# kingdwd/nlp-filter

Hardware: AMD Instinct MI355X
Metric: Gauss-Newton collocation-point updates/sec (higher is better)
Workload: dtype f64; 1 GPU; C2 van_der_pol: n=2, m=1, full_state p=2, N=100 (P=101, d=202), T=10, M=101; global_batch=1024, batch_per_gpu=1024, parallelism=dp1 (independent trajectories; RCCL broadcast of constants only)

## Files before the change

### nlp-filter_amd/csrc/mhe_core.h

```cpp
#pragma once
#include <hip/hip_runtime.h>
#include <math.h>
#include <stdint.h>
#include <stdlib.h>

#include "mhe.h"
#include "mhe_models.h"
#include "mhe_wave.h"

namespace mhe {

typedef double d4 __attribute__((ext_vector_type(4)));

#ifndef MHE_GN_MINW
#define MHE_GN_MINW 4
#endif
#ifndef MHE_NW
#define MHE_NW 8
#endif
constexpr int NW = MHE_NW;
constexpr int NTHREADS = NW * 64;
constexpr int MAX_NT = 13;
constexpr int MAX_SLOTS = (MAX_NT * (MAX_NT - 1) / 2 + NW - 1) / NW;

enum Mode { MODE_SOLVE = 0, MODE_ASSEMBLE = 1, MODE_LINSOLVE = 2, MODE_COV = 3 };

extern int g_opt_big_right_looking;
extern int g_opt_smem_pad;
extern int g_opt_lsm_group;

struct ConstLayout {
  size_t D, Dt, Phi, PhiT, cw, Qw, Pw, Rw, Cc, DA, DB, DAc, DBc, total;
};

__host__ __device__ inline size_t align256(size_t x) { return (x + 255) & ~size_t(255); }

constexpr size_t CONST_HEADER = 256;

__host__ __device__ inline ConstLayout const_layout(int P, int M, int n, int p, int NT) {
  ConstLayout L;
  size_t o = CONST_HEADER;
  const size_t ntiles = size_t(NT) * (NT + 1) / 2;
  L.D = o;    o = align256(o + sizeof(double) * P * P);
  L.Dt = o;   o = align256(o + sizeof(double) * P * P);
  L.Phi = o;  o = align256(o + sizeof(double) * M * P);
  L.PhiT = o; o = align256(o + sizeof(double) * M * P);
  L.cw = o;   o = align256(o + sizeof(double) * P);
  L.Qw = o;   o = align256(o + sizeof(double) * n * n);
  L.Pw = o;   o = align256(o + sizeof(double) * n * n);
  L.Rw = o;   o = align256(o + sizeof(double) * M * p * p);
  L.Cc = o;   o = align256(o + sizeof(double) * ntiles * 256);
  L.DA = o;   o = align256(o + sizeof(double) * ntiles * 256);
  L.DB = o;   o = align256(o + sizeof(double) * ntiles * 256);
  L.DAc = o;  o = align256(o + sizeof(double) * ntiles * 64);
  L.DBc = o;  o = align256(o + sizeof(double) * ntiles * 64);
  L.total = o;
  return L;
}

struct SmemLayout {
  int Xs, Vs, FtV, Es, FtE, GE, G, LAM, BV, YV, PB, HB, BAND, ZT, DT, RED, ROWM, UN, XO, ACT, GV, ZP, total;
};

__host__ __device__ inline int rnd2(int x) { return (x + 1) & ~1; }

constexpr int DTS = 272;
constexpr int LIS = 17;
constexpr int UNITS = 68;
constexpr int MFMA_NEG_A = 1;
__host__ __device__ constexpr int unit_row(int i) { return (i & 1) ? 51 - i : 16 - i; }

__host__ __device__ inline SmemLayout smem_layout(int P, int M, int n, int NT, bool nonlinear, bool bounded = false,
                                                  bool sb = false, bool cov = false) {
  SmemLayout S;
  int o = 0;
  const int dp = 16 * NT;
  S.Xs = o;   o += rnd2(P * n);
  S.Vs = o;   o += rnd2(P * n);
  S.FtV = o;  o += rnd2(P * n);
  S.Es = o;   o += rnd2(P * n * n);
  S.FtE = o;  o += rnd2(P * n * n);
  S.GE = o;   o += rnd2(M * n);
  S.G = o;    o += nonlinear ? rnd2(M * n * n) : 0;
  S.LAM = o;  o += rnd2(P * n);
  S.BV = o;   o += dp;
  S.YV = o;   o += dp;
  S.PB = o;   o += (sb ? 2 : 1) * (NT - 1) * 256;
  S.HB = o;   o += sb ? 2 * 256 : 0;
  S.BAND = o; o += sb ? (NT - 1) * 256 : 0;
  S.ZT = o;   o += sb ? 256 : 0;
  S.DT = o;   o += NT * DTS;
  S.RED = o;  o += 4 * NW + 8;
  S.ROWM = o; o += NW * 8;
  S.UN = o;   o += UNITS;
  S.XO = o;   o += bounded ? rnd2(P * n) : 0;
  S.ACT = o;  o += bounded ? dp / 2 : 0;
  S.GV = o;   o += bounded ? dp : 0;
  S.ZP = o;   o += cov ? dp * 16 : 0;
  S.total = o;
  return S;
}

struct GnArgs {
  const char* cbuf;
  int P, M, d, NT, ntiles, q, has_prior;
  int idx[8];
  double alpha;
  const double* X0;
  double* Xout;
  const double* U;
  long long ustride;
  const double* Y;
  const double* PAR;
  long long pstride;
  const double* x0;
  double* cost;
  int* iters;
  int* status;
  int max_iter;
  double tol;
  double* Hout;
  double* gout;
  const double* Hin;
  const double* gin;
  double* dout;
  unsigned long long* dbg;
  double huber_delta;
  int n_bounds;
  unsigned long long tag;
  int bidx[8];
  double blb[8], bub[8];
  double dpar[8];
  const double* Rw;
  long long rwstride;
  const double* PhiQ;
  int nq;
  double* cov;
  const double* md;
  long long mdstride;
  const double* Pw;
  long long pwstride;
  const double* Z0;
  double* Zout;
  double* lam;
  int nz, nc;
};

__device__ __forceinline__ const double* prior_weight(const GnArgs& a, const ConstLayout& CL, int b) {
  return a.Pw ? a.Pw + (long long)b * a.pwstride : (const double*)(a.cbuf + CL.Pw);
}

#ifdef MHE_DIAG
#define DIAG_DECL unsigned long long _dg[16] = {}; unsigned long long _dt = __builtin_amdgcn_s_memtime();
#define DIAG_MARK(i) do { const unsigned long long _n = __builtin_amdgcn_s_memtime(); _dg[i] += _n - _dt; _dt = _n; } while (0)
#define DIAG_FLUSH(b) do { if (threadIdx.x == 0 && a.dbg) for (int _i = 0; _i < 16; ++_i) a.dbg[(b) * 16 + _i] = _dg[_i]; } while (0)
#define DIAG_FDECL unsigned long long* _dg, unsigned long long& _dt
#define DIAG_FARGS _dg, _dt
#else
#define DIAG_DECL
#define DIAG_MARK(i) do { } while (0)
#define DIAG_FLUSH(b) do { } while (0)
#define DIAG_FDECL int
#define DIAG_FARGS 0
#endif

#ifndef MHE_KO
#define MHE_KO 0
#endif
#define KO(bit) ((MHE_KO >> (bit)) & 1)

__device__ __forceinline__ double readlane_d(double v, int lane) {
  const long long b = __double_as_longlong(v);
  const int lo = __builtin_amdgcn_readlane((int)b, lane);
  const int hi = __builtin_amdgcn_readlane((int)(b >> 32), lane);
  return __longlong_as_double(((long long)hi << 32) | (unsigned int)lo);
}

typedef unsigned int mhe_u2 __attribute__((ext_vector_type(2)));
__device__ __forceinline__ __amdgpu_buffer_rsrc_t cbuf_rsrc(const char* cbuf, size_t bytes) {
  return __builtin_amdgcn_make_buffer_rsrc((void*)cbuf, (short)0, (int)bytes, 0x00020000);
}
__device__ __forceinline__ double bload(__amdgpu_buffer_rsrc_t r, int voff, int soff) {
  const mhe_u2 v = __builtin_amdgcn_raw_buffer_load_b64(r, voff, soff, 0);
  return __builtin_bit_cast(double, v);
}


__device__ __forceinline__ void spread_dblock(double v, double (&o)[4]) {
  const double ev = dpp_d<0xA0>(v);
  const double od = dpp_d<0xF5>(v);
  const long long be = __double_as_longlong(ev), bo = __double_as_longlong(od);
  const auto el = __builtin_amdgcn_permlane16_swap((int)be, (int)be, false, false);
  const auto eh = __builtin_amdgcn_permlane16_swap((int)(be >> 32), (int)(be >> 32), false, false);
  const auto ol = __builtin_amdgcn_permlane16_swap((int)bo, (int)bo, false, false);
  const auto oh = __builtin_amdgcn_permlane16_swap((int)(bo >> 32), (int)(bo >> 32), false, false);
  o[0] = __longlong_as_double(((long long)eh[0] << 32) | (unsigned int)el[0]);
  o[2] = __longlong_as_double(((long long)eh[1] << 32) | (unsigned int)el[1]);
  o[1] = __longlong_as_double(((long long)oh[0] << 32) | (unsigned int)ol[0]);
  o[3] = __longlong_as_double(((long long)oh[1] << 32) | (unsigned int)ol[1]);
}

__device__ __forceinline__ double wave_max(double v) {
  v = fmax(v, dpp_d<0xB1>(v));
  v = fmax(v, dpp_d<0x4E>(v));
  v = fmax(v, dpp_d<0x141>(v));
  v = fmax(v, dpp_d<0x140>(v));
  v = pair_combine<1, true>(v);
  return pair_combine<2, true>(v);
}

template <bool SW = false>
__device__ __forceinline__ void block_reduce2(double* red, double& a, double& b, bool is_max) {
  const int lane = threadIdx.x & 63;
  int wave = threadIdx.x >> 6;
  if constexpr (SW) wave = __builtin_amdgcn_readfirstlane(wave);
  a = is_max ? wave_max(a) : wave_sum(a);
  b = is_max ? wave_max(b) : wave_sum(b);
  if (lane == 0) {
    red[2 * wave] = a;
    red[2 * wave + 1] = b;
  }
  __syncthreads();
  double ra = red[0], rb = red[1];
#pragma unroll
  for (int w = 1; w < NW; ++w) {
    ra = is_max ? fmax(ra, red[2 * w]) : ra + red[2 * w];
    rb = is_max ? fmax(rb, red[2 * w + 1]) : rb + red[2 * w + 1];
  }
  __syncthreads();
  a = ra;
  b = rb;
}

__device__ __forceinline__ int make_slot_table(int wave, int lane, int NT) {
  const int u = wave + NW * lane;
  if (lane >= MAX_SLOTS || u >= NT * (NT - 1) / 2) return -1;
  int J = 0, base = 0;
  while (u >= base + (NT - 1 - J)) {
    base += NT - 1 - J;
    ++J;
  }
  return (J + 1 + (u - base)) | (J << 16);
}

__device__ __forceinline__ int tile_index(int I, int J, int NT) { return J * NT - J * (J - 1) / 2 + (I - J); }

__device__ __forceinline__ int slot_ij(int stab, int s) { return __builtin_amdgcn_readlane(stab, s); }

__device__ __forceinline__ int slot_start(int j, int wave, int NT) {
  const int base = j * (NT - 1) - j * (j - 1) / 2;
  return base > wave ? (base - wave + NW - 1) / NW : 0;
}

struct ChainMap {
  unsigned short ij[NW][MAX_SLOTS];
  unsigned char pre[NW][16];
  unsigned char rows[MAX_NT][NW];
};

constexpr ChainMap make_chain_map(int NT) {
  ChainMap m = {};
  int rem[NW] = {}, nslot[NW] = {}, colc[MAX_NT][NW] = {};
  for (int w = 0; w < NW; ++w) {
    rem[w] = MAX_SLOTS;
    for (int s = 0; s < MAX_SLOTS; ++s) m.ij[w][s] = 0xffff;
  }
  int need = NT * (NT - 1) / 2 - (NW - 1) * MAX_SLOTS;
  for (int J = 0; J + 1 < NT; ++J) {
// ... 44 lines not shown

constexpr bool CHAIN_NW = NW == 8;
struct ChainMaps {
  ChainMap nt[MAX_NT + 1];
};
constexpr ChainMaps make_chain_maps() {
  ChainMaps a = {};
  for (int NT = 1; CHAIN_NW && NT <= MAX_NT; ++NT) a.nt[NT] = make_chain_map(NT);
  return a;
}

constexpr bool chain_map_ok(const ChainMap& m, int NT) {
  int seen[MAX_NT][MAX_NT] = {};
  for (int w = 0; w < NW; ++w) {
    int last = -1, rowc[MAX_NT] = {};
    bool ended = false;
    for (int s = 0; s < MAX_SLOTS; ++s) {
      const int v = m.ij[w][s];
      if (v == 0xffff) {
        ended = true;
        continue;
      }
      const int I = v & 0xff, J = v >> 8;
      if (ended || I <= J || I >= NT) return false;
      if ((J << 8 | I) <= last) return false;
      last = J << 8 | I;
      ++seen[I][J];
      ++rowc[J];
    }
    for (int J = 0; J + 1 < NT; ++J) {
      if (rowc[J] > (NT - 1 - J + NW - 1) / NW || rowc[J] != m.rows[J][w]) return false;
      if (m.pre[w][J + 1] - m.pre[w][J] != rowc[J]) return false;
    }
    if (m.pre[w][0] != 0) return false;
  }
  for (int I = 0; I < NT; ++I)
    for (int J = 0; J < NT; ++J)
      if (seen[I][J] != (I > J ? 1 : 0)) return false;
  for (int k = 0; k + 1 < NT; ++k) {
    for (int w = 1; w < NW; ++w) {
      int t0 = 0, tw = 0;
      for (int J = k + 1; J + 1 < NT; ++J) t0 += m.rows[J][0], tw += m.rows[J][w];
      if (tw < t0) return false;
    }
  }
  return true;
}
constexpr bool chain_maps_ok(const ChainMaps& a) {
  for (int NT = 1; NT <= MAX_NT; ++NT)
    if (!chain_map_ok(a.nt[NT], NT)) return false;
  return true;
}
constexpr ChainMaps CHAIN_MAPS_H = make_chain_maps();
static_assert(!CHAIN_NW || chain_maps_ok(CHAIN_MAPS_H),
              "panel-aware slot map: tile ownership, slot limit, row spread or slot order");
static __constant__ ChainMaps CHAIN_MAPS = CHAIN_MAPS_H;

constexpr int CHL_PRE = 16;
__device__ __forceinline__ int make_slot_table_chain(int wave, int lane, int NT) {
  const ChainMap& m = CHAIN_MAPS.nt[NT];
  if (lane >= CHL_PRE + 16) return -1;
  if (lane >= CHL_PRE) return m.pre[wave][lane - CHL_PRE];
  if (lane >= MAX_SLOTS) return -1;
  const int v = m.ij[wave][lane];
  return v == 0xffff ? -1 : (v & 0xff) | ((v >> 8) << 16);
}

__device__ __forceinline__ void init_units(double* un) {
  if (threadIdx.x < 64)
    for (int e = threadIdx.x; e < UNITS; e += 64) un[e] = (e == 16 || e == 51) ? 1.0 : 0.0;
}

template <int SLOTS = MAX_SLOTS>
__device__ __forceinline__ void init_rowmask(int* rowm, int wave, int lane, int stab) {
  unsigned m = 0;
#pragma unroll
  for (int s = 0; s < SLOTS; ++s) {
    const int IJ = slot_ij(stab, s);
    if (IJ >= 0 && (IJ & 0xffff) == lane) m |= 1u << s;
  }
  if (lane < 16) rowm[wave * 16 + lane] = (int)m;
}

constexpr int TPR = NW >= 8 ? 4 : 2;

__device__ __forceinline__ int opaque_tid() {
  int t = threadIdx.x;
  asm volatile("" : "+v"(t));
  return t;
}

template <int n>
__device__ __forceinline__ void dot_rows_part(const double* __restrict__ Mt, int ld, int row, int len, int part,
                                              const double* __restrict__ Xs, double (&acc)[n]) {
#pragma unroll
  for (int c = 0; c < n; ++c) acc[c] = 0.0;
  int j = part;
#pragma unroll 1
  for (; j + TPR * 7 < len; j += TPR * 8) {
    double m[8];
#pragma unroll
    for (int u = 0; u < 8; ++u) m[u] = Mt[(j + TPR * u) * ld + row];
#pragma unroll
    for (int u = 0; u < 8; ++u)
#pragma unroll
      for (int c = 0; c < n; ++c) acc[c] += m[u] * Xs[(j + TPR * u) * n + c];
  }
  for (; j < len; j += TPR) {
    const double mv = Mt[j * ld + row];
#pragma unroll
    for (int c = 0; c < n; ++c) acc[c] += mv * Xs[j * n + c];
  }
  static_assert(TPR == 4, "quad reductions below assume 4 lanes per row");
#pragma unroll
  for (int c = 0; c < n; ++c) acc[c] += dpp_d<0xB1>(acc[c]);
#pragma unroll
  for (int c = 0; c < n; ++c) acc[c] += dpp_d<0x4E>(acc[c]);
}

template <class DYN, bool HUBER = false>
__device__ __forceinline__ double node_row(const GnArgs& a, const ConstLayout& CL, const SmemLayout& SL, double* sm,
                                           int b, int k, const double (&dx)[DYN::n]) {
  constexpr int n = DYN::n, m = DYN::m;
  const double* cw = (const double*)(a.cbuf + CL.cw);
  const double* Qw = (const double*)(a.cbuf + CL.Qw);
  const double* Xs = sm + SL.Xs;
  double cost = 0.0;
  {
    double xk[n], uk[m > 0 ? m : 1], f[n], F[n * n];
#pragma unroll
    for (int c = 0; c < n; ++c) xk[c] = Xs[k * n + c];
    if (m > 0) {
      const double* U = a.U + (long long)b * a.ustride + (long long)k * m;
#pragma unroll
      for (int c = 0; c < m; ++c) uk[c] = U[c];
    }
    DYN::eval(xk, uk, a.dpar, f, F);
    double W[n], V[n];
#pragma unroll
    for (int c = 0; c < n; ++c) W[c] = a.alpha * dx[c] - f[c];
    const double ck = cw[k];
    double E[n * n];
    if constexpr (HUBER) {
      const double dl = a.huber_delta;
#pragma unroll
      for (int r = 0; r < n; ++r) {
        const double q = Qw[r * n + r];
        const double sr = sqrt(1.0 + W[r] * W[r] / (dl * dl));
        const double lam = ck * (q / sr);
        V[r] = lam * W[r];
        cost += ck * (2.0 * q * dl * dl * (sr - 1.0));
        sm[SL.LAM + k * n + r] = lam;
#pragma unroll
        for (int c = 0; c < n; ++c) E[r * n + c] = lam * F[r * n + c];
      }
    } else {
#pragma unroll
      for (int r = 0; r < n; ++r) {
        double s = 0.0;
#pragma unroll
        for (int c = 0; c < n; ++c) s += Qw[r * n + c] * W[c];
        V[r] = ck * s;
        cost += W[r] * V[r];
      }
#pragma unroll
      for (int r = 0; r < n; ++r)
#pragma unroll
// ... 110 lines not shown
      }
    }
    double* GE = sm + SL.GE + i * n;
#pragma unroll
    for (int c = 0; c < n; ++c) {
      double s = 0.0;
#pragma unroll
      for (int r = 0; r < p; ++r) s += H[r * n + c] * Re[r];
      GE[c] = s;
    }
    if (!MEAS::LINEAR) {
      double* G = sm + SL.G + i * n * n;
      double RH[p * n];
#pragma unroll
      for (int r = 0; r < p; ++r)
#pragma unroll
        for (int c = 0; c < n; ++c) {
          double s = 0.0;
#pragma unroll
          for (int t = 0; t < p; ++t) s += R[r * p + t] * H[t * n + c];
          RH[r * n + c] = s;
        }
#pragma unroll
      for (int r = 0; r < n; ++r)
#pragma unroll
        for (int c = 0; c < n; ++c) {
          double s = 0.0;
#pragma unroll
          for (int t = 0; t < p; ++t) s += H[t * n + r] * RH[t * n + c];
          G[r * n + c] = s;
        }
    }
  }
  return cost;
}

template <class DYN, class MEAS, bool NOISE = false, bool MHUBER = false>
__device__ __forceinline__ double meas_phase(const GnArgs& a, const ConstLayout& CL, const SmemLayout& SL, double* sm, int b,
                                             double* nzp = nullptr) {
  constexpr int n = DYN::n;
  const double* PhiT = (const double*)(a.cbuf + CL.PhiT);
  const double* Xs = sm + SL.Xs;
  double cost = 0.0;
  const int tid = opaque_tid();
  const int part = tid % TPR;
  for (int i0 = 0; i0 < a.M; i0 += NTHREADS / TPR) {
    const int i = i0 + tid / TPR;
    const int ii = i < a.M ? i : a.M - 1;
    double xi[n];
    dot_rows_part<n>(PhiT, a.M, ii, a.P, part, Xs, xi);
    if (part || i >= a.M) continue;
    cost += meas_row<DYN, MEAS, NOISE, MHUBER>(a, CL, SL, sm, b, i, xi, nzp);
  }
  return cost;
}

__device__ __forceinline__ double row_pair_sum(double v) {
  const long long b = __double_as_longlong(v);
  const auto l = __builtin_amdgcn_permlane16_swap((int)b, (int)b, false, false);
  const auto h = __builtin_amdgcn_permlane16_swap((int)(b >> 32), (int)(b >> 32), false, false);
  return __longlong_as_double(((long long)h[0] << 32) | (unsigned int)l[0]) +
         __longlong_as_double(((long long)h[1] << 32) | (unsigned int)l[1]);
}
__device__ __forceinline__ double upper_half(double v) {
  const long long b = __double_as_longlong(v);
  const auto l = __builtin_amdgcn_permlane32_swap((int)b, (int)b, false, false);
  const auto h = __builtin_amdgcn_permlane32_swap((int)(b >> 32), (int)(b >> 32), false, false);
  return __longlong_as_double(((long long)h[1] << 32) | (unsigned int)l[1]);
}

template <class DYN, class MEAS, bool HUBER = false, bool NOISE = false, bool MHUBER = false, bool SKIP = false>
__device__ __forceinline__ double node_meas_phase(const GnArgs& a, const ConstLayout& CL, const SmemLayout& SL,
                                                  double* sm, int b, DIAG_FDECL, double* nzp = nullptr) {
  constexpr int n = DYN::n;
  constexpr int ROWS = NTHREADS / TPR;
  if (a.P > ROWS || a.M > ROWS)
    return node_phase<DYN, HUBER>(a, CL, SL, sm, b) + meas_phase<DYN, MEAS, NOISE, MHUBER>(a, CL, SL, sm, b, nzp);
  const __amdgpu_buffer_rsrc_t rs = cbuf_rsrc(a.cbuf, CL.total);
  const double* Xs = sm + SL.Xs;
  const int tid = opaque_tid();
  if constexpr (SKIP)
    if (16 * __builtin_amdgcn_readfirstlane(tid >> 6) >= (a.P > a.M ? a.P : a.M)) return 0.0;
  const int part = (tid >> 4) & 3, r = (tid >> 6) * 16 + (tid & 15);
  const int kk = r < a.P ? r : a.P - 1, ii = r < a.M ? r : a.M - 1;
  double dx[n], xi[n];
#pragma unroll
  for (int c = 0; c < n; ++c) dx[c] = xi[c] = 0.0;
  const int len = a.P;
  int o1 = (int)CL.Dt + (part * a.P + kk) * 8, o2 = (int)CL.PhiT + (part * a.M + ii) * 8;
  const int s1 = TPR * a.P * 8, s2 = TPR * a.M * 8;
  int j = part;
#pragma unroll 1
  for (; j + TPR * 7 < len; j += TPR * 8) {
    double m1[8], m2[8];
#pragma unroll
    for (int u = 0; u < 8; ++u) {
      m1[u] = bload(rs, o1, u * s1);
      m2[u] = bload(rs, o2, u * s2);
    }
    o1 += 8 * s1;
    o2 += 8 * s2;
#pragma unroll
    for (int u = 0; u < 8; ++u)
#pragma unroll
      for (int c = 0; c < n; ++c) {
        const double x = Xs[(j + TPR * u) * n + c];
        dx[c] += m1[u] * x;
        xi[c] += m2[u] * x;
      }
  }
  for (; j < len; j += TPR) {
    const double m1 = bload(rs, o1, 0), m2 = bload(rs, o2, 0);
    o1 += s1;
    o2 += s2;
#pragma unroll
    for (int c = 0; c < n; ++c) {
      dx[c] += m1 * Xs[j * n + c];
      xi[c] += m2 * Xs[j * n + c];
    }
  }
  static_assert(TPR == 4, "the row reductions below assume 4 parts per row");
#pragma unroll
  for (int c = 0; c < n; ++c) {
    dx[c] = row_pair_sum(dx[c]);
    xi[c] = row_pair_sum(xi[c]);
  }
#pragma unroll
  for (int c = 0; c < n; ++c) {
    dx[c] += upper_half(dx[c]);
    xi[c] += upper_half(xi[c]);
  }
  DIAG_MARK(14);
  double cost = 0.0;
  if (part == 0) {
    if (r < a.P) cost += node_row<DYN, HUBER>(a, CL, SL, sm, b, r, dx);
    if (r < a.M) cost += meas_row<DYN, MEAS, NOISE, MHUBER>(a, CL, SL, sm, b, r, xi, nzp);
  }
  return cost;
}

template <class DYN, class MEAS, bool HUBER = false, bool NOISE = false, bool MHUBER = false, bool SKIP = false>
__device__ __forceinline__ double node_meas_phase(const GnArgs& a, const ConstLayout& CL, const SmemLayout& SL,
                                                  double* sm, int b, double* nzp = nullptr) {
  DIAG_DECL
  return node_meas_phase<DYN, MEAS, HUBER, NOISE, MHUBER, SKIP>(a, CL, SL, sm, b, DIAG_FARGS, nzp);
}

template <int n>
__device__ __forceinline__ double prior_cost(const GnArgs& a, const double* Pw, const double* Xs, int b) {
  double r0[n], cost = 0.0;
#pragma unroll
  for (int c = 0; c < n; ++c) r0[c] = Xs[c] - a.x0[(long long)b * n + c];
#pragma unroll
  for (int r = 0; r < n; ++r) {
    double t2 = 0.0;
#pragma unroll
    for (int c = 0; c < n; ++c) t2 += Pw[r * n + c] * r0[c];
    cost += r0[r] * t2;
  }
  return cost;
}

template <class DYN, bool PW = true, bool SKIP = false, bool OZ = false>
__device__ __forceinline__ double grad_phase(const GnArgs& a, const ConstLayout& CL, const SmemLayout& SL, double* sm, int b) {
  constexpr int n = DYN::n;
  const __amdgpu_buffer_rsrc_t rs = cbuf_rsrc(a.cbuf, CL.total);
  const double* Vs = sm + SL.Vs;
  const double* FtV = sm + SL.FtV;
  const double* GE = sm + SL.GE;
  const double* Xs = sm + SL.Xs;
  double* BV = sm + SL.BV;
  double cost = 0.0;
  const int dp = 16 * a.NT;
  const int tid = opaque_tid();
  constexpr int HP = TPR / 2;
  const int q = (tid >> 4) & 3, sub = q % HP;
  const bool phi = q >= HP;
  for (int j0 = 0; j0 < a.P; j0 += NTHREADS / TPR) {
    if constexpr (SKIP)
      if (j0 + 16 * __builtin_amdgcn_readfirstlane(tid >> 6) >= a.P) break;
    const int j = j0 + (tid >> 6) * 16 + (tid & 15);
    const int jj = j < a.P ? j : a.P - 1;
    const double* vec = phi ? GE : Vs;
    const int len = phi ? a.M : a.P;
    double s[n];
#pragma unroll
    for (int c = 0; c < n; ++c) s[c] = 0.0;
    int om = (int)(phi ? CL.Phi : CL.D) + (sub * a.P + jj) * 8;
    const int sm8 = HP * a.P * 8;
    int k = sub;
#pragma unroll 1
    for (; k + HP * 7 < len; k += HP * 8) {
      double mv[8];
#pragma unroll
      for (int u = 0; u < 8; ++u) mv[u] = bload(rs, om, u * sm8);
      om += 8 * sm8;
#pragma unroll
      for (int u = 0; u < 8; ++u)
#pragma unroll
        for (int c = 0; c < n; ++c) s[c] += mv[u] * vec[(k + HP * u) * n + c];
    }
    for (; k < len; k += HP) {
      const double mv = bload(rs, om, 0);
      om += sm8;
#pragma unroll
      for (int c = 0; c < n; ++c) s[c] += mv * vec[k * n + c];
    }
    static_assert(HP == 2, "the row reductions below assume TPR == 4");
#pragma unroll
    for (int c = 0; c < n; ++c) s[c] = row_pair_sum(s[c]);
    double o[n];
#pragma unroll
    for (int c = 0; c < n; ++c) o[c] = upper_half(s[c]);
    if (q != 0 || j >= a.P) continue;
    double gv[n];
#pragma unroll
    for (int c = 0; c < n; ++c) gv[c] = a.alpha * s[c] - FtV[j * n + c] - o[c];
    if (a.has_prior && j == 0) {
      const double* Pw = PW ? prior_weight(a, CL, b) : (const double*)(a.cbuf + CL.Pw);
      double r0[n];
#pragma unroll
      for (int c = 0; c < n; ++c) r0[c] = Xs[c] - a.x0[(long long)b * n + c];
#pragma unroll
      for (int r = 0; r < n; ++r) {
        double t2 = 0.0;
#pragma unroll
        for (int c = 0; c < n; ++c) t2 += Pw[r * n + c] * r0[c];
        gv[r] += t2;
        cost += r0[r] * t2;
      }
    }
#pragma unroll
    for (int c = 0; c < n; ++c) BV[j * n + c] = -gv[c];
  }
  double zero = 0.0;
  if constexpr (OZ) asm volatile("" : "+v"(zero));
  for (int t = a.d + tid; t < dp; t += NTHREADS) BV[t] = zero;
  return cost;
}

template <class DYN, class MEAS, bool HUBER = false>
__device__ __forceinline__ double h_element(const GnArgs& a, const double* Phi, const double* Es,
                                            const double* FtE, const double* G, double v, double da,
                                            double db, int row, int col, const double* D = nullptr,
                                            const double* LAM = nullptr) {
  constexpr int n = DYN::n;
  if (row < a.d && col < a.d) {
    const int j = row / n, aa = row - j * n;
    const int l = col / n, bb = col - l * n;
    if constexpr (HUBER) {
      if (aa == bb) {
        double s = 0.0;
        for (int k = 0; k < a.P; ++k) s += D[k * a.P + j] * LAM[k * n + aa] * D[k * a.P + l];
        v += a.alpha * a.alpha * s;
      }
    }
    v -= da * Es[(l * n + aa) * n + bb] + db * Es[(j * n + bb) * n + aa];
    if (j == l) v += FtE[(j * n + aa) * n + bb];
    if (!MEAS::LINEAR) {
      double s2 = 0.0;
      for (int i = 0; i < a.M; ++i) s2 += Phi[i * a.P + j] * Phi[i * a.P + l] * G[(i * n + aa) * n + bb];
      v += s2;
    }
  }
  return v;
}

template <int SLOTS, bool BOUNDED>
__device__ __forceinline__ void build_slots_n2(const GnArgs& a, const ConstLayout& CL, const SmemLayout& SL,
                                               double* sm, d4 (&acc)[SLOTS], int lane, int stab) {
  const __amdgpu_buffer_rsrc_t rs = cbuf_rsrc(a.cbuf, CL.total);
  const double* Es = sm + SL.Es;
  const int* ACT = (const int*)(sm + SL.ACT);
  double cn[4], an, bn;
  auto issue = [&](int s) {
    const int IJ = slot_ij(stab, s);
    const int ti = IJ < 0 ? 0 : tile_index(IJ & 0xffff, IJ >> 16, a.NT);
#pragma unroll
    for (int r = 0; r < 4; ++r) cn[r] = bload(rs, ti * 2048 + lane * 8, (int)CL.Cc + 512 * r);
    an = bload(rs, ti * 512 + lane * 8, (int)CL.DAc);
    bn = bload(rs, ti * 512 + lane * 8, (int)CL.DBc);
  };
  issue(0);
#pragma unroll
  for (int s = 0; s < SLOTS; ++s) {
    const double c[4] = {cn[0], cn[1], cn[2], cn[3]};
    const double av = an, bv = bn;
    if (s + 1 < SLOTS) issue(s + 1);
    const int IJ = slot_ij(stab, s);
// ... 1444 lines not shown
```

### nlp-filter_amd/csrc/mhe_general.h

```cpp

constexpr int FG_LDS_DOUBLES = 160 * 1024 / 8;

struct FgConst {
  ConstLayout C;
  size_t erow, ne, flag, rowe, eq, eqr, total;
};
__host__ __device__ inline FgConst fg_const_layout(int P, int M, int n, int NT, int nc) {
  FgConst L;
  L.C = const_layout(P, M, n, 1, NT);
  size_t o = L.C.total;
  const int Mr = M > 0 ? M : 1, ncr = nc > 0 ? nc : 1;
  L.erow = o; o = align256(o + sizeof(int) * (Mr + 1));
  L.ne = o;   o = align256(o + sizeof(int));
  L.flag = o; o = align256(o + sizeof(int) * Mr);
  L.rowe = o; o = align256(o + sizeof(int) * Mr);
  L.eq = o;   o = align256(o + sizeof(int) * 2 * ncr);
  L.eqr = o;  o = align256(o + sizeof(double) * ncr);
  L.total = o;
  L.C.total = o;
  return L;
}

struct FgSmem {
  SmemLayout S;
  int XE, ZS, GZ, HZZ, GZV, VP, MS, RW, LC, FLG, PHE, total;
};
__host__ __device__ inline FgSmem fg_smem_layout(int P, int EC, int n, int NT, int nz, int nc) {
  constexpr int NZX = MHE_MAX_EXTRA;
  FgSmem F;
  F.S = smem_layout(P, EC, n, NT, true);
  int o = F.S.total;
  const int K = nz + nc, KP = (K + 15) / 16 * 16, dp = 16 * NT;
  F.XE = o;  o += rnd2(EC * n);
  F.ZS = o;  o += NZX;
  F.GZ = o;  o += nz > 0 ? rnd2(EC * n * NZX) : 0;
  F.HZZ = o; o += nz > 0 ? EC * NZX * NZX : 0;
  F.GZV = o; o += nz > 0 ? EC * NZX : 0;
  F.VP = o;  o += KP * dp;
  F.MS = o;  o += rnd2(K * K);
  F.RW = o;  o += rnd2(K);
  F.LC = o;  o += rnd2(K);
  F.FLG = o; o += 2;
  F.PHE = o; o += rnd2(EC * P);
  F.total = o;
  return F;
}

__host__ __device__ inline int fg_epoch_cap(int P, int M, int n, int NT, int nz, int nc) {
  constexpr int NZX = MHE_MAX_EXTRA;
  const int fixed = fg_smem_layout(P, 0, n, NT, nz, nc).total + 8;
  const int per = n + n * n + n + P + (nz > 0 ? n * NZX + NZX * NZX + NZX : 0);
  const int cap = fixed < FG_LDS_DOUBLES ? (FG_LDS_DOUBLES - fixed) / per : 0;
  return M < cap ? M : cap;
}

template <class DYN, class MEAS>
__device__ __forceinline__ double fg_resid(const GnArgs& ae, const FgConst& FC, const FgSmem& FS, double* sm, int b,
                                           int E, int Mf) {
  constexpr int n = DYN::n, NZX = MHE_MAX_EXTRA, q = MEAS::q;
  const ConstLayout& CL = FC.C;
  const SmemLayout& SL = FS.S;
  const int nz = ae.nz;
  double cost = node_phase<DYN>(ae, CL, SL, sm, b);
  const int tid = opaque_tid();
  {
    const double* PhiET = (const double*)(ae.cbuf + CL.PhiT);
    const double* Xs = sm + SL.Xs;
    for (int e = tid; e < E; e += NTHREADS) {
      double xe[n];
#pragma unroll
      for (int c = 0; c < n; ++c) xe[c] = 0.0;
      for (int j = 0; j < ae.P; ++j) {
        const double ph = PhiET[(size_t)j * Mf + e];
#pragma unroll
        for (int c = 0; c < n; ++c) xe[c] += ph * Xs[j * n + c];
      }
#pragma unroll
      for (int c = 0; c < n; ++c) sm[FS.XE + e * n + c] = xe[c];
    }
    for (int t = tid; t < E * n * n; t += NTHREADS) sm[SL.G + t] = 0.0;
    for (int t = tid; t < E * n; t += NTHREADS) sm[SL.GE + t] = 0.0;
    if (nz > 0) {
      for (int t = tid; t < E * n * NZX; t += NTHREADS) sm[FS.GZ + t] = 0.0;
      for (int t = tid; t < E * NZX * NZX; t += NTHREADS) sm[FS.HZZ + t] = 0.0;
      for (int t = tid; t < E * NZX; t += NTHREADS) sm[FS.GZV + t] = 0.0;
    }
  }
  __syncthreads();
  {
    const int* erow = (const int*)(ae.cbuf + FC.erow);
    const double* Rw = ae.Rw ? ae.Rw + (long long)b * ae.rwstride : (const double*)(ae.cbuf + CL.Rw);
    const double* Zs = sm + FS.ZS;
    const int u = tid & 7;
    for (int e = tid >> 3; e < E; e += NTHREADS / 8) {
      const double* xe = sm + FS.XE + e * n;
      double* G = sm + SL.G + e * n * n;
      double* ge = sm + SL.GE + e * n;
      double* Gz = sm + FS.GZ + e * n * NZX;
      double* Hzz = sm + FS.HZZ + e * NZX * NZX;
      double* gz = sm + FS.GZV + e * NZX;
      const int i1 = erow[e + 1];
      for (int i = erow[e]; i < i1; ++i) {
        const double R = Rw[i];
        if (R == 0.0) continue;
        const double* PR = ae.PAR + (long long)b * ae.pstride + (long long)i * q;
        double h, gs[7];
        int id[7];
        MEAS::eval_slots([&](int c) { return c < n ? xe[c] : Zs[c - n]; }, PR, nz, h, id, gs);
#pragma unroll
        for (int k1 = 0; k1 < 7; ++k1)
#pragma unroll
          for (int k2 = k1 + 1; k2 < 7; ++k2)
            if (id[k1] >= 0 && id[k2] == id[k1]) {
              gs[k1] += gs[k2];
              id[k2] = -1;
            }
#pragma unroll
        for (int k1 = 0; k1 < 7; ++k1)
          if (gs[k1] == 0.0) id[k1] = -1;
        const double ev = ae.Y[(long long)b * Mf + i] - h;
        const double Re = R * ev;
        if (u == 0) cost += ev * Re;
        int ia = -1;
        double ga = 0.0;
#pragma unroll
        for (int k1 = 0; k1 < 7; ++k1)
          if (u == k1) {
            ia = id[k1];
            ga = gs[k1];
          }
        if (ia >= 0) {
          if (ia < n) ge[ia] += ga * Re;
          else gz[ia - n] += ga * Re;
#pragma unroll
          for (int v = 0; v < 7; ++v) {
            if (id[v] < 0) continue;
            const int ib = id[v];
            const double w2 = R * (ga * gs[v]);
            if (ia < n && ib < n) G[ia * n + ib] += w2;
            else if (ia < n) Gz[ia * NZX + (ib - n)] += w2;
            else if (ib >= n) Hzz[(ia - n) * NZX + (ib - n)] += w2;
          }
        }
        wave_lds_sync();
      }
    }
  }
  __syncthreads();
  cost += grad_phase<DYN, true>(ae, CL, SL, sm, b);
  return cost;
}

template <int n, int SLOTS>
__device__ __forceinline__ bool fg_border(const GnArgs& ae, const FgConst& FC, const FgSmem& FS, double* sm,
                                          d4 (&acc)[SLOTS], int wave, int lane, int stab, int b, int E) {
  constexpr int NZX = MHE_MAX_EXTRA;
  const SmemLayout& SL = FS.S;
  const int nz = ae.nz, nc = ae.nc, K = nz + nc, KP = (K + 15) / 16 * 16;
  const int NT = ae.NT, dp = 16 * NT, d = ae.d, P = ae.P;
  const double* PhiE = (const double*)(ae.cbuf + FC.C.Phi);
  const int* eq = (const int*)(ae.cbuf + FC.eq);
  const double* eqr = (const double*)(ae.cbuf + FC.eqr);
  double* VP = sm + FS.VP;
  double* YV = sm + SL.YV;
  double* Ms = sm + FS.MS;
  double* rw = sm + FS.RW;
  double* lc = sm + FS.LC;
  int* flg = (int*)(sm + FS.FLG);
  auto vat = [&](int i, int c) -> double& { return VP[(c >> 4) * dp * 16 + (i >> 4) * 256 + (i & 15) * 16 + (c & 15)]; };
  for (int t = threadIdx.x; t < KP * dp; t += NTHREADS) {
    const int c = t / dp, i = t - c * dp;
    double v = 0.0;
    if (i < d && c < K) {
      if (c < nz) {
        const int j = i / n, ca = i - j * n;
        for (int e = 0; e < E; ++e) v += PhiE[(size_t)e * P + j] * sm[FS.GZ + (e * n + ca) * NZX + c];
      } else {
        if (eq[2 * (c - nz)] == i) v += 1.0;
        if (eq[2 * (c - nz) + 1] == i) v -= 1.0;
      }
    }
    vat(i, c) = v;
  }
  if (threadIdx.x == 0) flg[0] = 0;
  __syncthreads();
  for (int p0 = 0; p0 < KP; p0 += 16) {
    d4 unused = {0.0, 0.0, 0.0, 0.0};
    fwd_sweep_panel<SLOTS, true>(NT, sm + SL.DT, VP + p0 * dp, acc, wave, lane, stab, unused);
    __syncthreads();
  }
  for (int t = wave; t < K * K + K; t += NW) {
    const bool isr = t >= K * K;
    const int r = isr ? t - K * K : t / K, c = isr ? 0 : t - (t / K) * K;
    if (!isr && c > r) continue;
    double s = 0.0;
    for (int i = lane; i < dp; i += 64) s += vat(i, r) * (isr ? YV[i] : vat(i, c));
    s = wave_sum(s);
    if (lane == 0) {
      double base = 0.0;
      if (isr) {
        if (r < nz) {
          for (int e = 0; e < E; ++e) base += sm[FS.GZV + e * NZX + r];
        } else {
          const int ia = eq[2 * (r - nz)], ib = eq[2 * (r - nz) + 1];
          base = -(sm[SL.Xs + ia] - (ib >= 0 ? sm[SL.Xs + ib] : 0.0) - eqr[r - nz]);
        }
        rw[r] = base - s;
      } else {
        if (r < nz && c < nz)
          for (int e = 0; e < E; ++e) base += sm[FS.HZZ + e * NZX * NZX + r * NZX + c];
        Ms[r * K + c] = base - s;
        Ms[c * K + r] = base - s;
      }
    }
  }
  __syncthreads();
  if (wave == 0) {
    bool bad = false;
    for (int t = lane; t < K * K; t += 64) bad |= !isfinite(Ms[t]);
    big_ldl_factor(Ms, lc, K, lane);
    if (lane < K) bad |= !isfinite(Ms[lane * K + lane]);
    if (lane == 0) big_ldl_solve(Ms, rw, K, 1);
    if (bad) flg[0] = 1;
  }
  __syncthreads();
  if (flg[0] != 0) return false;
  for (int i = threadIdx.x; i < dp; i += NTHREADS) {
    double s = YV[i];
    for (int c = 0; c < K; ++c) s -= vat(i, c) * rw[c];
    YV[i] = s;
  }
  if (ae.lam)
// ... 128 lines not shown
```

### nlp-filter_amd/csrc/mhe_gn.hip

```cpp
#include <cstdio>
#include <string.h>

#include "mhe_core.h"

namespace mhe {

__global__ void k_copy_consts(int P, int M, int n, int p, int NT, const double* D, const double* cw,
                              const double* Phi, const double* Qw, const double* Rw, const double* Pw,
                              char* cbuf) {
  const ConstLayout CL = const_layout(P, M, n, p, NT);
  double* oD = (double*)(cbuf + CL.D);
  double* oDt = (double*)(cbuf + CL.Dt);
  double* oPhi = (double*)(cbuf + CL.Phi);
  double* oPhiT = (double*)(cbuf + CL.PhiT);
  const int gid = blockIdx.x * blockDim.x + threadIdx.x;
  const int stride = gridDim.x * blockDim.x;
  for (int e = gid; e < P * P; e += stride) {
    const int k = e / P, j = e % P;
    oD[e] = D[e];
    oDt[j * P + k] = D[e];
  }
  for (int e = gid; e < M * P; e += stride) {
    const int i = e / P, j = e % P;
    oPhi[e] = Phi[e];
    oPhiT[j * M + i] = Phi[e];
  }
  for (int e = gid; e < P; e += stride) ((double*)(cbuf + CL.cw))[e] = cw[e];
  for (int e = gid; e < n * n; e += stride) {
    ((double*)(cbuf + CL.Qw))[e] = Qw[e];
    ((double*)(cbuf + CL.Pw))[e] = Pw ? Pw[e] : 0.0;
  }
  for (int e = gid; e < M * p * p; e += stride) ((double*)(cbuf + CL.Rw))[e] = Rw[e];
}

__global__ void k_big_init(BigArgs a, int batch) {
  const int b = blockIdx.x * blockDim.x + threadIdx.x;
  if (b < batch) {
    const bool ok = *(const unsigned long long*)a.cbuf == a.tag;
    a.state[b] = ok ? BIG_RUNNING : MHE_STATUS_BAD_CONSTANTS;
    a.iters[b] = 0;
    if (!ok) a.cost[b] = NAN;
  }
}

__global__ void k_big_finish(int batch, int* state) {
  const int b = blockIdx.x * blockDim.x + threadIdx.x;
  if (b < batch && state[b] == BIG_RUNNING) state[b] = MHE_STATUS_MAX_ITER;
}

__global__ void k_big_consts(int P, int M, int n, int p, const double* D, const double* cw, const double* Qw,
                             const double* Rw, const double* Pw, char* cbuf) {
  const BigConst CL = big_const_layout(P, M, n, p);
  const int gid = blockIdx.x * blockDim.x + threadIdx.x, stride = gridDim.x * blockDim.x;
  double* oD = (double*)(cbuf + CL.D);
  double* oDt = (double*)(cbuf + CL.Dt);
  double* oDCD = (double*)(cbuf + CL.DCD);
  for (int e = gid; e < P * P; e += stride) {
    const int k = e / P, j = e % P;
    oD[e] = D[e];
    oDt[j * P + k] = D[e];
    const int lo = k < j ? k : j, hi = k < j ? j : k;
    double s = 0.0;
    for (int t = 0; t < P; ++t) s += D[t * P + lo] * cw[t] * D[t * P + hi];
    oDCD[e] = s;
  }
  for (int e = gid; e < P; e += stride) ((double*)(cbuf + CL.cw))[e] = cw[e];
  for (int e = gid; e < n * n; e += stride) {
    ((double*)(cbuf + CL.Qw))[e] = Qw[e];
    ((double*)(cbuf + CL.Pw))[e] = Pw ? Pw[e] : 0.0;
  }
  for (int e = gid; e < M * p * p; e += stride) ((double*)(cbuf + CL.Rw))[e] = Rw[e];
}

struct EqPairs {
  int v[2 * MHE_MAX_EQ];
  double r[MHE_MAX_EQ];
};
__global__ void k_big_eq_consts(int P, int M, int n, int p, int nc, EqPairs e, char* cbuf) {
  const BigConst CL = big_const_layout(P, M, n, p, nc);
  int* o = (int*)(cbuf + CL.eq);
  double* orr = (double*)(cbuf + CL.eqr);
  for (int i = threadIdx.x; i < 2 * nc; i += blockDim.x) o[i] = e.v[i];
  for (int i = threadIdx.x; i < nc; i += blockDim.x) orr[i] = e.r[i];
}

__global__ void k_big_epoch_flags(int P, int M, int n, int p, const double* Phi, char* cbuf) {
  const BigConst CL = big_const_layout(P, M, n, p);
  int* flag = (int*)(cbuf + CL.flag);
  for (int i = blockIdx.x * blockDim.x + threadIdx.x; i < M; i += gridDim.x * blockDim.x) {
    int f = (i == 0);
    if (!f)
      for (int j = 0; j < P; ++j)
        if (__double_as_longlong(Phi[(size_t)i * P + j]) != __double_as_longlong(Phi[(size_t)(i - 1) * P + j])) {
          f = 1;
          break;
        }
    flag[i] = f;
  }
}

__global__ void k_big_epoch_scan(int P, int M, int n, int p, char* cbuf) {
  const BigConst CL = big_const_layout(P, M, n, p);
  const int* flag = (const int*)(cbuf + CL.flag);
  int* erow = (int*)(cbuf + CL.erow);
  int E = 0;
  for (int i = 0; i < M; ++i)
    if (flag[i]) erow[E++] = i;
  erow[E] = M;
  *(int*)(cbuf + CL.ne) = E;
}

__global__ void k_big_epoch_rows(int P, int M, int n, int p, const double* Phi, char* cbuf) {
  const BigConst CL = big_const_layout(P, M, n, p);
  const int* erow = (const int*)(cbuf + CL.erow);
  const int E = *(const int*)(cbuf + CL.ne);
// ... 64 lines not shown
    const double v = e < E ? Phi[(size_t)erow[e] * P + j] : 0.0;
    PhiE[(size_t)e * P + j] = v;
    PhiET[(size_t)j * M + e] = v;
  }
}

__global__ void k_write_tag(unsigned long long* p, unsigned long long tag) { *p = tag; }

int g_opt_big_right_looking = 0;
int g_opt_smem_pad = 0;

}

using namespace mhe;

#ifdef MHE_DIAG
static unsigned long long* g_dbg = nullptr;
#endif

namespace {

const PairOps* find_pair(const mhe_dims* dm) {
  const PairOps* ops = pairs_vdp(dm->dyn_model, dm->meas_model);
#ifndef MHE_FAST_BUILD
  if (!ops) ops = pairs_integrators(dm->dyn_model, dm->meas_model);
  if (!ops) ops = pairs_gnss(dm->dyn_model, dm->meas_model);
  if (!ops) ops = pairs_vehicles(dm->dyn_model, dm->meas_model);
  if (!ops) ops = pairs_autocar(dm->dyn_model, dm->meas_model);
  if (!ops) ops = pairs_receivers(dm->dyn_model, dm->meas_model);
#endif
  return ops;
}

int check_dims(const mhe_dims* dm, int* NT_out) {
  if (!dm) return MHE_ERR_NULL;
  if (dm->struct_size != (int32_t)sizeof(mhe_dims)) return MHE_ERR_DIMS;
  int n, m, p, q;
  bool lin;
  if (!dyn_info(dm->dyn_model, n, m)) return MHE_ERR_MODEL;
  if (!meas_info(dm->meas_model, n, p, q, lin)) return MHE_ERR_MODEL;
  if (dm->n != n || dm->m != m || dm->p != p || dm->q != q) return MHE_ERR_DIMS;
  if (dm->N < 1 || dm->M < 0 || !(dm->T > 0.0)) return MHE_ERR_DIMS;
  if (dm->dyn_cost != MHE_COST_L2 && dm->dyn_cost != MHE_COST_HUBER) return MHE_ERR_MODEL;
  if (dm->dyn_cost == MHE_COST_HUBER && !(dm->huber_delta > 0.0)) return MHE_ERR_DIMS;
  if (dm->n_bounds < 0 || dm->n_bounds > 8) return MHE_ERR_DIMS;
  for (int i = 0; i < dm->n_bounds; ++i)
    if (dm->bound_idx[i] < 0 || dm->bound_idx[i] >= n || !(dm->bound_lb[i] <= dm->bound_ub[i])) return MHE_ERR_DIMS;
  if (dm->meas_model == MHE_MEAS_VEHICLE_PSEUDORANGE && dm->dyn_model != MHE_DYN_VEHICLE_GNSS) return MHE_ERR_DIMS;
  for (int i = 0; i < 4; ++i)
    if ((dm->meas_model == MHE_MEAS_PSEUDORANGE && (dm->meas_idx[i] < 0 || dm->meas_idx[i] >= n)) ||
        (dm->meas_model == MHE_MEAS_RANGE_3D && i < 3 && (dm->meas_idx[i] < 0 || dm->meas_idx[i] >= n)))
      return MHE_ERR_DIMS;
  const int P = dm->N + 1;
  if (dm->n_extra < 0 || dm->n_extra > MHE_MAX_EXTRA || dm->n_eq < 0 || dm->n_extra + dm->n_eq > MHE_MAX_EQ)
    return MHE_ERR_DIMS;
  if (dm->n_extra > 0 && dm->meas_model != MHE_MEAS_MIXED) return MHE_ERR_DIMS;
  if (dm->n_eq > 0) {
    if (!dm->eq_idx) return MHE_ERR_NULL;
    for (int i = 0; i < dm->n_eq; ++i) {
      const int ia = dm->eq_idx[2 * i], ib = dm->eq_idx[2 * i + 1];
      if (ia < 0 || ia >= P * n || ib < -1 || ib >= P * n || ia == ib) return MHE_ERR_DIMS;
    }
  }
  if (dm->n_bounds > 0 && (dm->n_eq > 0 || dm->n_extra > 0)) return MHE_ERR_UNSUPPORTED;
  int NT = (P * n + 15) / 16;
  if (is_big(dm)) NT = n * big_pp(P) / 16;
  if (NT_out) *NT_out = NT;
  return MHE_OK;
}

size_t const_total_bytes(const mhe_dims* dm, int NT) {
  if (is_big(dm)) return big_const_layout(dm->N + 1, dm->M, dm->n, dm->p, dm->n_eq).total;
  if (fg_eligible(dm)) return fg_const_layout(dm->N + 1, dm->M, dm->n, NT, dm->n_eq).total;
  return const_layout(dm->N + 1, dm->M, dm->n, dm->p, NT).total;
}

unsigned long long const_tag(const mhe_dims* dm, int NT) {
  unsigned long long h = 1469598103934665603ull;
  auto mix = [&h](long long x) {
    h ^= (unsigned long long)x;
    h *= 1099511628211ull;
  };
  const long long v[] = {0x4D4845, is_big(dm) ? 1 : fg_eligible(dm) ? 2 : 0, dm->N, dm->n, dm->m, dm->p, dm->M, dm->q, dm->dyn_model,
                         dm->meas_model, dm->has_prior, dm->dyn_cost, NT, dm->n_eq, dm->n_extra};
  for (long long x : v) mix(x);
  if (dm->n_eq > 0 && dm->eq_idx)
    for (int i = 0; i < 2 * dm->n_eq; ++i) mix(dm->eq_idx[i]);
  for (int i = 0; i < dm->n_eq; ++i) {
    const double r = (dm->eq_rhs ? dm->eq_rhs[i] : 0.0) + 0.0;
    long long bits;
    memcpy(&bits, &r, sizeof bits);
    mix(bits);
  }
  return h | 1ull;
}

EqPairs eq_pairs(const mhe_dims* dm) {
  EqPairs e = {};
  for (int i = 0; i < 2 * dm->n_eq; ++i) e.v[i] = dm->eq_idx[i];
  for (int i = 0; i < dm->n_eq; ++i) e.r[i] = dm->eq_rhs ? dm->eq_rhs[i] : 0.0;
  return e;
}

int build_big_consts(const mhe_dims* dm, const double* D, const double* cw, const double* Phi, const double* Qw,
                     const double* Rw, const double* Pw, char* cbuf, hipStream_t st) {
  const int P = dm->N + 1;
  hipLaunchKernelGGL(k_big_consts, dim3(256), dim3(256), 0, st, P, dm->M, dm->n, dm->p, D, cw, Qw, Rw, Pw, cbuf);
  if (dm->M > 0) {
    hipLaunchKernelGGL(k_big_epoch_flags, dim3((dm->M + 255) / 256), dim3(256), 0, st, P, dm->M, dm->n, dm->p, Phi,
                       cbuf);
    hipLaunchKernelGGL(k_big_epoch_scan, dim3(1), dim3(1), 0, st, P, dm->M, dm->n, dm->p, cbuf);
    hipLaunchKernelGGL(k_big_epoch_rows, dim3(256), dim3(256), 0, st, P, dm->M, dm->n, dm->p, Phi, cbuf);
  }
  if (dm->n_eq > 0)
    hipLaunchKernelGGL(k_big_eq_consts, dim3(1), dim3(128), 0, st, P, dm->M, dm->n, dm->p, dm->n_eq, eq_pairs(dm),
                       cbuf);
  return hipGetLastError() == hipSuccess ? MHE_OK : MHE_ERR_HIP;
}

template <class A>
void set_dims(A& a, const mhe_dims* dm, const void* cbuf, int NT) {
  a.cbuf = (const char*)cbuf;
  a.P = dm->N + 1;
  a.M = dm->M;
  a.NT = NT;
  a.q = dm->q;
  a.has_prior = dm->has_prior;
  a.alpha = 2.0 / dm->T;
  a.huber_delta = dm->huber_delta;
  a.n_bounds = dm->n_bounds;
  a.tag = const_tag(dm, NT);
  for (int i = 0; i < 8; ++i) {
    a.idx[i] = dm->meas_idx[i];
    a.bidx[i] = dm->bound_idx[i];
    a.blb[i] = dm->bound_lb[i];
    a.bub[i] = dm->bound_ub[i];
    a.dpar[i] = dm->dyn_par[i];
  }
  a.nz = dm->n_extra;
  a.nc = dm->n_eq;
}

template <class A>
void set_point(A& a, const mhe_solve_args* at) {
  a.U = at->U; a.ustride = at->u_bstride; a.Y = at->Y; a.PAR = at->PAR; a.pstride = at->par_bstride; a.x0 = at->x0;
  a.Rw = at->Rw; a.rwstride = at->rw_bstride; a.md = at->meas_delta; a.mdstride = at->md_bstride;
  a.Pw = at->Pw; a.pwstride = at->pw_bstride;
}

GnArgs make_args(const mhe_dims* dm, const void* cbuf, int NT) {
  GnArgs a = {};
#ifdef MHE_DIAG
  a.dbg = g_dbg;
#endif
  set_dims(a, dm, cbuf, NT);
  a.d = a.P * dm->n;
  a.ntiles = NT * (NT + 1) / 2;
  return a;
}

int build_fg_consts(const mhe_dims* dm, int NT, const PairOps* ops, const double* D, const double* cw,
                    const double* Phi, const double* Qw, const double* Rw, const double* Pw, char* cbuf,
                    hipStream_t st) {
  const int P = dm->N + 1;
  hipLaunchKernelGGL(k_fg_consts, dim3(64), dim3(256), 0, st, P, dm->M, dm->n, NT, dm->n_eq, eq_pairs(dm), D, cw, Qw,
                     Rw, Pw, cbuf);
  int rc = ops->build_cc(dm, NT, D, cw, Phi, Qw, Rw, Pw, cbuf, st);
// ... 748 lines not shown
```

Baseline: 692.7 million GN collocation-point updates/s.

## Pre-swizzle D/Phi into per-lane interleaved streams for 128-bit matvec loads

```diff
diff --git a/nlp-filter_amd/csrc/mhe_core.h b/nlp-filter_amd/csrc/mhe_core.h
--- a/nlp-filter_amd/csrc/mhe_core.h
+++ b/nlp-filter_amd/csrc/mhe_core.h
@@ -20,6 +20,8 @@
 #endif
 constexpr int NW = MHE_NW;
 constexpr int NTHREADS = NW * 64;
+constexpr int TPR = NW >= 8 ? 4 : 2;
+constexpr int MV_ROWS = NTHREADS / TPR;
 constexpr int MAX_NT = 13;
 constexpr int MAX_SLOTS = (MAX_NT * (MAX_NT - 1) / 2 + NW - 1) / NW;
 
@@ -30,14 +32,30 @@
 extern int g_opt_lsm_group;
 
 struct ConstLayout {
-  size_t D, Dt, Phi, PhiT, cw, Qw, Pw, Rw, Cc, DA, DB, DAc, DBc, total;
+  size_t D, Dt, Phi, PhiT, cw, Qw, Pw, Rw, Cc, DA, DB, DAc, DBc, NMS, GRS, total;
+  int nmu, grv;
 };
 
 __host__ __device__ inline size_t align256(size_t x) { return (x + 255) & ~size_t(255); }
 
 constexpr size_t CONST_HEADER = 256;
-
-__host__ __device__ inline ConstLayout const_layout(int P, int M, int n, int p, int NT) {
+constexpr int CONST_LAYOUT_REV = 2;
+
+constexpr int STREAM_PIECE = 64 * 16;
+__host__ __device__ inline int nms_terms(int P, int M) {
+  return (P <= MV_ROWS && M <= MV_ROWS) ? (P + TPR - 1) / TPR : 0;
+}
+__host__ __device__ inline int grs_pairs(int P, int M) { return ((P > M ? P : M) + 3) / 4; }
+__host__ __device__ inline int grs_passes(int P) { return (P + MV_ROWS - 1) / MV_ROWS; }
+
+#ifndef MHE_MV_STREAMS
+#define MHE_MV_STREAMS 3
+#endif
+__host__ __device__ constexpr bool mv_stream(int n, int bit) {
+  return (n == 2 || n == 4) && ((MHE_MV_STREAMS >> bit) & 1);
+}
+
+__host__ __device__ inline ConstLayout const_layout(int P, int M, int n, int p, int NT, bool streams = true) {
   ConstLayout L;
   size_t o = CONST_HEADER;
   const size_t ntiles = size_t(NT) * (NT + 1) / 2;
@@ -54,6 +72,10 @@
   L.DB = o;   o = align256(o + sizeof(double) * ntiles * 256);
   L.DAc = o;  o = align256(o + sizeof(double) * ntiles * 64);
   L.DBc = o;  o = align256(o + sizeof(double) * ntiles * 64);
+  L.nmu = streams && mv_stream(n, 0) ? nms_terms(P, M) : 0;
+  L.grv = streams && mv_stream(n, 1) ? grs_pairs(P, M) : 0;
+  L.NMS = o;  o = align256(o + size_t(STREAM_PIECE) * NW * L.nmu);
+  L.GRS = o;  o = align256(o + size_t(STREAM_PIECE) * NW * L.grv * grs_passes(P));
   L.total = o;
   return L;
 }
@@ -184,6 +206,12 @@
   const mhe_u2 v = __builtin_amdgcn_raw_buffer_load_b64(r, voff, soff, 0);
   return __builtin_bit_cast(double, v);
 }
+typedef unsigned int mhe_u4 __attribute__((ext_vector_type(4)));
+typedef double d2 __attribute__((ext_vector_type(2)));
+__device__ __forceinline__ d2 bload2(__amdgpu_buffer_rsrc_t r, int voff, int soff) {
+  const mhe_u4 v = __builtin_amdgcn_raw_buffer_load_b128(r, voff, soff, 0);
+  return __builtin_bit_cast(d2, v);
+}
 
 
 __device__ __forceinline__ void spread_dblock(double v, double (&o)[4]) {
@@ -394,7 +422,6 @@
   if (lane < 16) rowm[wave * 16 + lane] = (int)m;
 }
 
-constexpr int TPR = NW >= 8 ? 4 : 2;
 
 __device__ __forceinline__ int opaque_tid() {
   int t = threadIdx.x;
@@ -671,44 +698,73 @@
   if constexpr (SKIP)
     if (16 * __builtin_amdgcn_readfirstlane(tid >> 6) >= (a.P > a.M ? a.P : a.M)) return 0.0;
   const int part = (tid >> 4) & 3, r = (tid >> 6) * 16 + (tid & 15);
-  const int kk = r < a.P ? r : a.P - 1, ii = r < a.M ? r : a.M - 1;
   double dx[n], xi[n];
 #pragma unroll
   for (int c = 0; c < n; ++c) dx[c] = xi[c] = 0.0;
   const int len = a.P;
-  int o1 = (int)CL.Dt + (part * a.P + kk) * 8, o2 = (int)CL.PhiT + (part * a.M + ii) * 8;
-  const int s1 = TPR * a.P * 8, s2 = TPR * a.M * 8;
-  int j = part;
+  if constexpr (mv_stream(n, 0)) {
+    int o = (int)CL.NMS + __builtin_amdgcn_readfirstlane(tid >> 6) * CL.nmu * STREAM_PIECE + (tid & 63) * 16;
+    int j = part;
 #pragma unroll 1
-  for (; j + TPR * 7 < len; j += TPR * 8) {
-    double m1[8], m2[8];
-#pragma unroll
-    for (int u = 0; u < 8; ++u) {
-      m1[u] = bload(rs, o1, u * s1);
-      m2[u] = bload(rs, o2, u * s2);
-    }
-    o1 += 8 * s1;
-    o2 += 8 * s2;
-#pragma unroll
-    for (int u = 0; u < 8; ++u)
+    for (; j + TPR * 7 < len; j += TPR * 8) {
+      d2 m[8];
+#pragma unroll
+      for (int u = 0; u < 8; ++u) m[u] = bload2(rs, o, u * STREAM_PIECE);
+      o += 8 * STREAM_PIECE;
+#pragma unroll
+      for (int u = 0; u < 8; ++u)
+#pragma unroll
+        for (int c = 0; c < n; ++c) {
+          const double x = Xs[(j + TPR * u) * n + c];
+          dx[c] += m[u].x * x;
+          xi[c] += m[u].y * x;
+        }
+    }
+    for (; j < len; j += TPR) {
+      const d2 m = bload2(rs, o, 0);
+      o += STREAM_PIECE;
 #pragma unroll
       for (int c = 0; c < n; ++c) {
-        const double x = Xs[(j + TPR * u) * n + c];
-        dx[c] += m1[u] * x;
-        xi[c] += m2[u] * x;
-      }
-  }
-  for (; j < len; j += TPR) {
-    const double m1 = bload(rs, o1, 0), m2 = bload(rs, o2, 0);
-    o1 += s1;
-    o2 += s2;
-#pragma unroll
-    for (int c = 0; c < n; ++c) {
-      dx[c] += m1 * Xs[j * n + c];
-      xi[c] += m2 * Xs[j * n + c];
-    }
-  }
-  static_assert(TPR == 4, "the row reductions below assume 4 parts per row");
+        dx[c] += m.x * Xs[j * n + c];
+        xi[c] += m.y * Xs[j * n + c];
+      }
+    }
+  } else {
+    const int kk = r < a.P ? r : a.P - 1, ii = r < a.M ? r : a.M - 1;
+    int o1 = (int)CL.Dt + (part * a.P + kk) * 8, o2 = (int)CL.PhiT + (part * a.M + ii) * 8;
+    const int s1 = TPR * a.P * 8, s2 = TPR * a.M * 8;
+    int j = part;
+#pragma unroll 1
+    for (; j + TPR * 7 < len; j += TPR * 8) {
+      double m1[8], m2[8];
+#pragma unroll
+      for (int u = 0; u < 8; ++u) {
+        m1[u] = bload(rs, o1, u * s1);
+        m2[u] = bload(rs, o2, u * s2);
+      }
+      o1 += 8 * s1;
+      o2 += 8 * s2;
+#pragma unroll
+      for (int u = 0; u < 8; ++u)
+#pragma unroll
+        for (int c = 0; c < n; ++c) {
+          const double x = Xs[(j + TPR * u) * n + c];
+          dx[c] += m1[u] * x;
+          xi[c] += m2[u] * x;
+        }
+    }
+    for (; j < len; j += TPR) {
+      const double m1 = bload(rs, o1, 0), m2 = bload(rs, o2, 0);
+      o1 += s1;
+      o2 += s2;
+#pragma unroll
+      for (int c = 0; c < n; ++c) {
+        dx[c] += m1 * Xs[j * n + c];
+        xi[c] += m2 * Xs[j * n + c];
+      }
+    }
+  }
+  static_assert(TPR == 4, "the row reductions below and the NMS stream assume 4 parts per row");
 #pragma unroll
   for (int c = 0; c < n; ++c) {
     dx[c] = row_pair_sum(dx[c]);
@@ -750,7 +806,7 @@
   return cost;
 }
 
-template <class DYN, bool PW = true, bool SKIP = false, bool OZ = false>
+template <class DYN, bool PW = true, bool SKIP = false, bool OZ = false, bool STREAM = true>
 __device__ __forceinline__ double grad_phase(const GnArgs& a, const ConstLayout& CL, const SmemLayout& SL, double* sm, int b) {
   constexpr int n = DYN::n;
   const __amdgpu_buffer_rsrc_t rs = cbuf_rsrc(a.cbuf, CL.total);
@@ -775,25 +831,57 @@
     double s[n];
 #pragma unroll
     for (int c = 0; c < n; ++c) s[c] = 0.0;
-    int om = (int)(phi ? CL.Phi : CL.D) + (sub * a.P + jj) * 8;
-    const int sm8 = HP * a.P * 8;
     int k = sub;
+    if constexpr (STREAM && mv_stream(n, 1)) {
+      int og = (int)CL.GRS + (j0 / MV_ROWS * NW + __builtin_amdgcn_readfirstlane(tid >> 6)) * CL.grv * STREAM_PIECE +
+               (tid & 63) * 16;
 #pragma unroll 1
-    for (; k + HP * 7 < len; k += HP * 8) {
-      double mv[8];
-#pragma unroll
-      for (int u = 0; u < 8; ++u) mv[u] = bload(rs, om, u * sm8);
-      om += 8 * sm8;
-#pragma unroll
-      for (int u = 0; u < 8; ++u)
-#pragma unroll
-        for (int c = 0; c < n; ++c) s[c] += mv[u] * vec[(k + HP * u) * n + c];
-    }
-    for (; k < len; k += HP) {
-      const double mv = bload(rs, om, 0);
-      om += sm8;
-#pragma unroll
-      for (int c = 0; c < n; ++c) s[c] += mv * vec[k * n + c];
+      for (; k + HP * 7 < len; k += HP * 8) {
+        d2 mv[4];
+#pragma unroll
+        for (int u = 0; u < 4; ++u) mv[u] = bload2(rs, og, u * STREAM_PIECE);
+        og += 4 * STREAM_PIECE;
+#pragma unroll
+        for (int u = 0; u < 4; ++u) {
+#pragma unroll
+          for (int c = 0; c < n; ++c) s[c] += mv[u].x * vec[(k + HP * 2 * u) * n + c];
+#pragma unroll
+          for (int c = 0; c < n; ++c) s[c] += mv[u].y * vec[(k + HP * (2 * u + 1)) * n + c];
+        }
+      }
+      for (; k + HP < len; k += HP * 2) {
+        const d2 mv = bload2(rs, og, 0);
+        og += STREAM_PIECE;
+#pragma unroll
+        for (int c = 0; c < n; ++c) s[c] += mv.x * vec[k * n + c];
+#pragma unroll
+        for (int c = 0; c < n; ++c) s[c] += mv.y * vec[(k + HP) * n + c];
+      }
+      if (k < len) {
+        const double mv = bload(rs, og, 0);
+#pragma unroll
+        for (int c = 0; c < n; ++c) s[c] += mv * vec[k * n + c];
+      }
+    } else {
+      int om = (int)(phi ? CL.Phi : CL.D) + (sub * a.P + jj) * 8;
+      const int sm8 = HP * a.P * 8;
+#pragma unroll 1
+      for (; k + HP * 7 < len; k += HP * 8) {
+        double mv[8];
+#pragma unroll
+        for (int u = 0; u < 8; ++u) mv[u] = bload(rs, om, u * sm8);
+        om += 8 * sm8;
+#pragma unroll
+        for (int u = 0; u < 8; ++u)
+#pragma unroll
+          for (int c = 0; c < n; ++c) s[c] += mv[u] * vec[(k + HP * u) * n + c];
+      }
+      for (; k < len; k += HP) {
+        const double mv = bload(rs, om, 0);
+        om += sm8;
+#pragma unroll
+        for (int c = 0; c < n; ++c) s[c] += mv * vec[k * n + c];
+      }
     }
     static_assert(HP == 2, "the row reductions below assume TPR == 4");
 #pragma unroll
diff --git a/nlp-filter_amd/csrc/mhe_general.h b/nlp-filter_amd/csrc/mhe_general.h
--- a/nlp-filter_amd/csrc/mhe_general.h
+++ b/nlp-filter_amd/csrc/mhe_general.h
@@ -7,7 +7,7 @@
 };
 __host__ __device__ inline FgConst fg_const_layout(int P, int M, int n, int NT, int nc) {
   FgConst L;
-  L.C = const_layout(P, M, n, 1, NT);
+  L.C = const_layout(P, M, n, 1, NT, false);
   size_t o = L.C.total;
   const int Mr = M > 0 ? M : 1, ncr = nc > 0 ? nc : 1;
   L.erow = o; o = align256(o + sizeof(int) * (Mr + 1));
@@ -147,7 +147,7 @@
     }
   }
   __syncthreads();
-  cost += grad_phase<DYN, true>(ae, CL, SL, sm, b);
+  cost += grad_phase<DYN, true, false, false, false>(ae, CL, SL, sm, b);
   return cost;
 }
 
diff --git a/nlp-filter_amd/csrc/mhe_gn.hip b/nlp-filter_amd/csrc/mhe_gn.hip
--- a/nlp-filter_amd/csrc/mhe_gn.hip
+++ b/nlp-filter_amd/csrc/mhe_gn.hip
@@ -31,6 +31,24 @@
     ((double*)(cbuf + CL.Pw))[e] = Pw ? Pw[e] : 0.0;
   }
   for (int e = gid; e < M * p * p; e += stride) ((double*)(cbuf + CL.Rw))[e] = Rw[e];
+  double* oN = (double*)(cbuf + CL.NMS);
+  for (int e = gid; e < NW * CL.nmu * 64; e += stride) {
+    const int lane = e & 63, u = (e >> 6) % CL.nmu, w = (e >> 6) / CL.nmu;
+    const int j = (lane >> 4) + TPR * u, r = 16 * w + (lane & 15);
+    const int kk = r < P ? r : P - 1, ii = r < M ? r : M - 1;
+    oN[2 * e] = j < P ? D[kk * P + j] : 0.0;
+    oN[2 * e + 1] = j < P && M > 0 ? Phi[ii * P + j] : 0.0;
+  }
+  double* oG = (double*)(cbuf + CL.GRS);
+  for (int e = gid; e < grs_passes(P) * NW * CL.grv * 64; e += stride) {
+    const int lane = e & 63, v = (e >> 6) % CL.grv, pw = (e >> 6) / CL.grv;
+    const int q = lane >> 4, node = 16 * pw + (lane & 15), jj = node < P ? node : P - 1;
+    const bool phi = q >= TPR / 2;
+    const double* T = phi ? Phi : D;
+    const int len = phi ? M : P, k0 = q % (TPR / 2) + 4 * v, k1 = k0 + 2;
+    oG[2 * e] = k0 < len ? T[k0 * P + jj] : 0.0;
+    oG[2 * e + 1] = k1 < len ? T[k1 * P + jj] : 0.0;
+  }
 }
 
 __global__ void k_big_init(BigArgs a, int batch) {
@@ -261,7 +279,7 @@
     h *= 1099511628211ull;
   };
   const long long v[] = {0x4D4845, is_big(dm) ? 1 : fg_eligible(dm) ? 2 : 0, dm->N, dm->n, dm->m, dm->p, dm->M, dm->q, dm->dyn_model,
-                         dm->meas_model, dm->has_prior, dm->dyn_cost, NT, dm->n_eq, dm->n_extra};
+                         dm->meas_model, dm->has_prior, dm->dyn_cost, NT, dm->n_eq, dm->n_extra, CONST_LAYOUT_REV, NW};
   for (long long x : v) mix(x);
   if (dm->n_eq > 0 && dm->eq_idx)
     for (int i = 0; i < 2 * dm->n_eq; ++i) mix(dm->eq_idx[i]);
```

Result: faster. 712.1 million GN collocation-point updates/s (median of 6 runs) (+2.8%).
